# aliftffd/ViT-vs-Raw-IQ

Measured on AMD Instinct MI355X. Metric: IQ frames/sec training (fwd+loss+bwd+clip+AdamW), higher is better.
Workload: dtype bf16; 1 GPU; ViT-Tiny/16 224x224 C=1 19cls (BASELINE configs[1]); config_id=B, per_gpu_batch=256, global_batch=256, parallelism=dp1, hipgraph=True

## Files before the change

vit-vs-raw-iq_amd/csrc/common.h:

```cpp
#pragma once
#include <hip/hip_runtime.h>
#include <stdint.h>

#include "../../include/iqvit.h"

typedef __bf16 bf16;
typedef __attribute__((ext_vector_type(8))) __bf16 bf16x8;
typedef __attribute__((ext_vector_type(4))) __bf16 bf16x4;
typedef __attribute__((ext_vector_type(4))) short s16x4;
typedef __attribute__((ext_vector_type(8))) short s16x8;
typedef __attribute__((ext_vector_type(4))) float f32x4;
typedef __attribute__((ext_vector_type(4))) uint32_t u32x4;
typedef __attribute__((address_space(3))) void lds_void_t;
typedef __attribute__((address_space(1))) const void gbl_cvoid_t;

#define IQ_OK 0
#define IQ_ERR_ARG 1
#define IQ_ERR_UNSUPPORTED 2
#define IQ_ERR_LAUNCH 3

#define IQ_WAVE 64

static inline int iq_launch_status() {
  hipError_t e = hipGetLastError();
  return e == hipSuccess ? IQ_OK : IQ_ERR_LAUNCH;
}

__device__ __forceinline__ float bf2f(bf16 v) { return (float)v; }
__device__ __forceinline__ bf16 f2bf(float v) { return (bf16)v; }

__device__ __forceinline__ void unpack8(const bf16x8& v, float* f) {
#pragma unroll
  for (int i = 0; i < 8; ++i) f[i] = (float)v[i];
}
__device__ __forceinline__ bf16x8 pack8(const float* f) {
  bf16x8 v;
#pragma unroll
  for (int i = 0; i < 8; ++i) v[i] = (bf16)f[i];
  return v;
}

struct IqRng {
  uint64_t seed;
  uint32_t step;
  uint32_t site;
  const uint32_t* step_dev;
};

__device__ __forceinline__ IqRng rng_resolve(IqRng r) {
  if (r.step_dev) r.step = *r.step_dev;
  return r;
}

#ifndef IQ_PHILOX_ROUNDS
#define IQ_PHILOX_ROUNDS 7
#endif
__device__ __forceinline__ u32x4 philox4x32(uint32_t c0, uint32_t c1, uint32_t c2, uint32_t c3,
                                            uint32_t k0, uint32_t k1) {
  const uint32_t M0 = 0xD2511F53u, M1 = 0xCD9E8D57u, W0 = 0x9E3779B9u, W1 = 0xBB67AE85u;
#pragma unroll
  for (int r = 0; r < IQ_PHILOX_ROUNDS; ++r) {
    const uint64_t p0 = (uint64_t)M0 * (uint64_t)c0;
    const uint64_t p1 = (uint64_t)M1 * (uint64_t)c2;
    const uint32_t n0 = (uint32_t)(p1 >> 32) ^ c1 ^ k0, n1 = (uint32_t)p1;
    const uint32_t n2 = (uint32_t)(p0 >> 32) ^ c3 ^ k1, n3 = (uint32_t)p0;
    c0 = n0; c1 = n1; c2 = n2; c3 = n3;
    k0 += W0; k1 += W1;
  }
  u32x4 o = {c0, c1, c2, c3};
  return o;
}

__device__ __forceinline__ float u24(uint32_t w) { return (float)(w >> 8) * 0x1p-24f; }
__device__ __forceinline__ float u24_open(uint32_t w) { return (float)((w >> 8) + 1u) * 0x1p-24f; }
__device__ __forceinline__ void box_muller(uint32_t a, uint32_t b, float& g0, float& g1) {
  const float r = sqrtf(-2.f * logf(u24_open(a)));
  float sn, cs;
  sincospif(2.f * u24(b), &sn, &cs);
  g0 = r * cs;
  g1 = r * sn;
}

__device__ __forceinline__ uint32_t dropout_keep8(const IqRng& r, uint64_t group, uint32_t thresh) {
  u32x4 b = philox4x32((uint32_t)group, (uint32_t)(group >> 32), r.site, r.step,
                          (uint32_t)r.seed, (uint32_t)(r.seed >> 32));
  uint32_t m = 0;
#pragma unroll
  for (int i = 0; i < 4; ++i) {
    m |= ((b[i] & 0xFFFFu) >= thresh ? 1u : 0u) << (2 * i);
    m |= ((b[i] >> 16) >= thresh ? 1u : 0u) << (2 * i + 1);
  }
  return m;
}

__host__ __device__ inline uint32_t dropout_thresh(float p) {
  float t = p * 65536.0f + 0.5f;
  if (t < 0.f) t = 0.f;
  if (t > 65535.f) t = 65535.f;
  return (uint32_t)t;
}
__host__ __device__ inline float dropout_scale(float p) {
  uint32_t t = dropout_thresh(p);
  return 65536.0f / (65536.0f - (float)t);
}

inline bool dropout_unpack(const iq_dropout_t* d, int* on, IqRng* rng, uint32_t* thresh, float* dscale) {
  *on = 0; *rng = IqRng{0, 0, 0, nullptr}; *thresh = 0; *dscale = 1.f;
  if (!d || !(d->p > 0.f)) return true;
  *on = 1;
  *rng = IqRng{d->seed, d->step, d->site, d->step_dev};
  *thresh = dropout_thresh(d->p);
  *dscale = dropout_scale(d->p);
  return d->p < 1.f;
}

constexpr int vmcnt_imm(int n) { return (n & 15) | ((n >> 4) << 14) | 0x0F70; }

__device__ __forceinline__ int xcd_remap(int bid, int nwg) {
  const int NX = 8;
  int q = nwg / NX, r = nwg % NX;
  int xcd = bid % NX, idx = bid / NX;
  int base = (xcd < r) ? xcd * (q + 1) : r * (q + 1) + (xcd - r) * q;
  return base + idx;
}

// ... 11 lines not shown
```

vit-vs-raw-iq_amd/csrc/ffn_chain.hip:

```cpp
#include <stdlib.h>

#include <type_traits>

#include "common.h"
#include "iqvit.h"
#include "prof.h"

namespace {

constexpr int FC_CHUNK = 64, FC_NS = 3, FC_MAXW = 7;

struct FfnChainParams {
  const bf16* X1; const bf16* W1; const bf16* W2;
  const float* b1; const float* b2; const float* gamma; const float* beta;
  bf16* H; bf16* Z; bf16* X; float* mean; float* rstd;
  uint32_t* gate;
  int M, F;
  float eps;
  int drop1_on, drop2_on; IqRng rng1, rng2; uint32_t thresh1, thresh2; float dscale1, dscale2;
  const bf16* A0; const bf16* W0; const bf16* R0; const float* b0; const float* gamma0; const float* beta0;
  bf16* Z0; bf16* X1out; float* mean0; float* rstd0;
  int drop0_on; IqRng rng0; uint32_t thresh0; float dscale0;
  const bf16* Wq; const float* bq; bf16* Yq;
};

template <int CPR> __device__ __forceinline__ int fc_swz(int row, int ch) {
  return CPR == 16 ? (ch ^ (row & 15)) : CPR == 8 ? (ch ^ ((row >> 1) & 7)) : ((ch & ~7) | ((ch & 7) ^ ((row >> 1) & 7)));
}
template <int OFF>
__device__ __forceinline__ void lds_read128(bf16x8& dst, uint32_t addr) {
  asm volatile("ds_read_b128 %0, %1 offset:%2" : "=v"(dst) : "v"(addr), "n"(OFF));
}
#define FC_LGKM_WAIT(N)                                  \
  do {                                                   \
    asm volatile("s_waitcnt lgkmcnt(%0)" ::"n"(N) : "memory"); \
    __builtin_amdgcn_sched_barrier(0);                   \
  } while (0)

__device__ __forceinline__ int fc_kperm(int g) { return ((g & 1) << 1) | (g >> 1); }

template <int D, int NW, int RG, bool DROP1, int MODE>
__global__ __launch_bounds__(NW * 64, 2) void ffn_chain_fwd_kernel(const FfnChainParams p) {
  constexpr int RW = 16 * RG;
  constexpr bool PRE = MODE >= 1, POST = MODE == 2;
  constexpr int XCPR = D / 8;
  constexpr int KS1 = D / 32;
  constexpr int NT2 = D / 16, NP2 = NT2 / 2;
  constexpr int W1_BYTES = FC_CHUNK * D * 2, W2_BYTES = D * FC_CHUNK * 2, SLOT = W1_BYTES + W2_BYTES;
  constexpr int W1_PIECES = W1_BYTES / 1024, PIECES = SLOT / 1024;
  constexpr int PPW = (PIECES + NW - 1) / NW;
  static_assert(PPW + 8 * RG < 64, "counted vmcnt");
  extern __shared__ __attribute__((aligned(16))) unsigned char smem[];
  const int tid = threadIdx.x, lane = tid & 63;
  const int wave = __builtin_amdgcn_readfirstlane(tid >> 6);
  constexpr int nwave = NW;
  const int g = lane >> 4, c16 = lane & 15;
  const bool odd = (g & 1) != 0;
  const int F = p.F;
  const int nchunk = F / FC_CHUNK;
  const long row0 = ((long)blockIdx.x * nwave + wave) * RW;
  const bool have = row0 < p.M;

  auto issue_chunk = [&](int c) {
    unsigned char* slot = smem + (c % FC_NS) * SLOT;
    const char* base1 = reinterpret_cast<const char*>(p.W1 + (long)c * FC_CHUNK * D);
    const char* base2 = reinterpret_cast<const char*>(p.W2 + (long)c * FC_CHUNK);
    int ln = lane;
    asm volatile("" : "+v"(ln));
#pragma unroll
    for (int i = 0; i < PPW; ++i) {
      const int pc = min(wave + i * NW, PIECES - 1);
      const int lin = pc * 64 + ln;
      unsigned off;
      if (pc < W1_PIECES) {
        const int r = lin / XCPR, sl = lin - r * XCPR;
        const int q = fc_swz<XCPR>(r, sl);
        off = (unsigned)((r * D + ((q & ~3) | fc_kperm(q & 3)) * 8) * 2);
      } else {
        const int l2 = lin - W1_PIECES * 64;
        const int r = l2 >> 3, sl = l2 & 7;
        const int q = fc_swz<8>(r, sl);
        off = (unsigned)((r * F + ((q & ~3) | fc_kperm(q & 3)) * 8) * 2);
      }
      const char* base = pc < W1_PIECES ? base1 : base2;
      __builtin_amdgcn_global_load_lds((gbl_cvoid_t*)(base + off), (lds_void_t*)(slot + pc * 1024), 16, 0, 0);
    }
  };
  constexpr int NBQ = 3 * D / FC_CHUNK, NQ = (NBQ + 1) / 2;
  static_assert(2 * W1_BYTES == SLOT, "two projection blocks fill a ring slot");
  const int ntot = nchunk + (POST ? NQ : 0);
  auto issue_any = [&](int c) {
    if (!POST || c < nchunk) { issue_chunk(c); return; }
    const int q = c - nchunk;
    unsigned char* slot = smem + (c % FC_NS) * SLOT;
    int ln = lane;
    asm volatile("" : "+v"(ln));
#pragma unroll
    for (int i = 0; i < PPW; ++i) {
      const int pc = min(wave + i * NW, PIECES - 1);
      const int lin = pc * 64 + ln;
      const int r = lin / XCPR, sl = lin - r * XCPR;
      const int qq = fc_swz<XCPR>(r & 63, sl);
      const int grow = min(q * 2 * FC_CHUNK + r, 3 * D - 1);
      const unsigned off = (unsigned)((grow * D + ((qq & ~3) | fc_kperm(qq & 3)) * 8) * 2);
      __builtin_amdgcn_global_load_lds((gbl_cvoid_t*)(reinterpret_cast<const char*>(p.Wq) + off), (lds_void_t*)(slot + pc * 1024), 16, 0, 0);
    }
  };
  constexpr int NB0 = D / FC_CHUNK;
  if (PRE) {
    constexpr int PRE_PIECES = NB0 * W1_PIECES, PRE_PPW = (PRE_PIECES + NW - 1) / NW;
    static_assert(NB0 * W1_BYTES <= 2 * SLOT, "projection weight blocks fit ring slots 1 and 2");
#pragma unroll
    for (int i = 0; i < PRE_PPW; ++i) {
      const int pc = min(wave + i * NW, PRE_PIECES - 1);
      const int lin = pc * 64 + lane;
      const int r = lin / XCPR, sl = lin - r * XCPR;
      const int q = fc_swz<XCPR>(r & 63, sl);
      const unsigned off = (unsigned)((r * D + ((q & ~3) | fc_kperm(q & 3)) * 8) * 2);
      __builtin_amdgcn_global_load_lds((gbl_cvoid_t*)(reinterpret_cast<const char*>(p.W0) + off),
                                       (lds_void_t*)(smem + SLOT + pc * 1024), 16, 0, 0);
    }
  }
  issue_chunk(0);
  if (!PRE && ntot > 1) issue_any(1);

  bf16x8 xf[RG][KS1];
  {
    const bf16* src = PRE ? p.A0 : p.X1;
#pragma unroll
    for (int rg = 0; rg < RG; ++rg) {
      const long r = min(row0 + rg * 16 + c16, (long)p.M - 1);
#pragma unroll
      for (int ks = 0; ks < KS1; ++ks)
        xf[rg][ks] = have ? *reinterpret_cast<const bf16x8*>(src + r * D + 32 * ks + 8 * fc_kperm(g)) : bf16x8{};
    }
  }
  bf16x8 res0[PRE ? RG : 1][PRE ? KS1 : 1];
  if (PRE) {
#pragma unroll
    for (int rg = 0; rg < RG; ++rg) {
      const long r = min(row0 + rg * 16 + c16, (long)p.M - 1);
#pragma unroll
      for (int jp = 0; jp < KS1; ++jp)
        res0[rg][jp] = have ? *reinterpret_cast<const bf16x8*>(p.R0 + r * D + 32 * jp + 8 * fc_kperm(g)) : bf16x8{};
    }
  }
  const IqRng rng1 = DROP1 ? rng_resolve(p.rng1) : p.rng1;
  const IqRng rng2 = p.drop2_on ? rng_resolve(p.rng2) : p.rng2;
  float* b1s = reinterpret_cast<float*>(smem + FC_NS * SLOT);
  float* vecs = b1s + F;
  for (int i = tid; i < F / 4; i += NW * 64) reinterpret_cast<f32x4*>(b1s)[i] = reinterpret_cast<const f32x4*>(p.b1)[i];
  for (int i = tid; i < (PRE ? 6 : 3) * (D / 4); i += NW * 64) {
    const int v = i / (D / 4), j = i - v * (D / 4);
    const float* src = v == 0 ? p.b2 : v == 1 ? p.gamma : v == 2 ? p.beta : v == 3 ? p.b0 : v == 4 ? p.gamma0 : p.beta0;
    reinterpret_cast<f32x4*>(vecs)[i] = reinterpret_cast<const f32x4*>(src)[j];
  }
  if (POST)
    for (int i = tid; i < 3 * D / 4; i += NW * 64) reinterpret_cast<f32x4*>(vecs + 6 * D)[i] = reinterpret_cast<const f32x4*>(p.bq)[i];
  asm volatile("s_waitcnt vmcnt(0)" ::: "memory");
#pragma unroll
  for (int rg = 0; rg < RG; ++rg)
#pragma unroll
    for (int ks = 0; ks < KS1; ++ks) asm volatile("" : "+v"(xf[rg][ks]));
  if (PRE) {
#pragma unroll
    for (int rg = 0; rg < RG; ++rg)
#pragma unroll
      for (int jp = 0; jp < KS1; ++jp) asm volatile("" : "+v"(res0[rg][jp]));
  }

  const uint32_t lds0 = (uint32_t)(uintptr_t)(lds_void_t*)smem;
  constexpr int W1_KMASK = XCPR == 24 ? 1 : KS1 - 1;
  uint32_t w1off[KS1], w2off[2];
  auto w1at = [&](int ks) -> uint32_t { return w1off[ks & W1_KMASK] + (XCPR == 24 ? 128u * (uint32_t)(ks >> 1) : 0u); };
#pragma unroll
  for (int ks = 0; ks < KS1; ++ks) w1off[ks] = (uint32_t)(c16 * (D * 2) + fc_swz<XCPR>(c16, 4 * (ks & W1_KMASK) + g) * 16);
#pragma unroll
  for (int jp = 0; jp < 2; ++jp) w2off[jp] = (uint32_t)(W1_BYTES + c16 * 128 + fc_swz<8>(c16, 4 * jp + g) * 16);

  if (PRE) {
    __syncthreads();
    if (have) {
      const IqRng rng0 = p.drop0_on ? rng_resolve(p.rng0) : p.rng0;
      bf16x8 zb[RG][KS1];
#pragma unroll
      for (int b = 0; b < NB0; ++b) {
#pragma unroll
        for (int jp = 0; jp < 2; ++jp) {
          const int col = 32 * (2 * b + jp) + (odd ? 16 + 4 * (g - 1) : 4 * g);
          f32x4 acc1[RG][2];
#pragma unroll
          for (int rg = 0; rg < RG; ++rg) { acc1[rg][0] = f32x4{0.f, 0.f, 0.f, 0.f}; acc1[rg][1] = f32x4{0.f, 0.f, 0.f, 0.f}; }
          bf16x8 wp[2][2];
          const uint32_t blk = lds0 + SLOT + b * W1_BYTES;
          auto read_w0 = [&](int ks, bf16x8 (&dst)[2]) {
            const uint32_t a0 = blk + w1at(ks);
            if (jp == 0) { lds_read128<0 * 16 * D * 2>(dst[0], a0); lds_read128<1 * 16 * D * 2>(dst[1], a0); }
            else { lds_read128<2 * 16 * D * 2>(dst[0], a0); lds_read128<3 * 16 * D * 2>(dst[1], a0); }
          };
          read_w0(0, wp[0]);
#pragma unroll
          for (int ks = 0; ks < KS1; ++ks) {
            if (ks + 1 < KS1) { read_w0(ks + 1, wp[(ks + 1) & 1]); FC_LGKM_WAIT(2); }
            else FC_LGKM_WAIT(0);
#pragma unroll
            for (int t = 0; t < 2; ++t) {
#pragma unroll
              for (int rg = 0; rg < RG; ++rg)
                acc1[rg][t] = __builtin_amdgcn_mfma_f32_16x16x32_bf16(wp[ks & 1][t], xf[rg][ks], acc1[rg][t], 0, 0, 0);
            }
            __builtin_amdgcn_sched_barrier(0);
          }
          const f32x4 b_lo = *reinterpret_cast<const f32x4*>(vecs + 3 * D + col), b_hi = *reinterpret_cast<const f32x4*>(vecs + 3 * D + col + 4);
#pragma unroll
          for (int rg = 0; rg < RG; ++rg) {
            float w[8];
#pragma unroll
            for (int r = 0; r < 4; ++r) {
              const float va = acc1[rg][0][r], vb = acc1[rg][1][r];
              const auto sw = __builtin_amdgcn_permlane16_swap(__float_as_uint(va), __float_as_uint(vb), false, false);
              w[r] = __uint_as_float(sw[0]) + b_lo[r];
              w[4 + r] = __uint_as_float(sw[1]) + b_hi[r];
            }
            const long grow = row0 + rg * 16 + c16;
            if (p.drop0_on) {
              const uint32_t keep = dropout_keep8(rng0, (uint64_t)(grow * D + col) >> 3, p.thresh0);
#pragma unroll
              for (int e = 0; e < 8; ++e) w[e] = ((keep >> e) & 1u) ? w[e] * p.dscale0 : 0.f;
            }
#pragma unroll
            for (int e = 0; e < 8; ++e) w[e] += (float)res0[rg][2 * b + jp][e];
            zb[rg][2 * b + jp] = pack8(w);
            if (grow < p.M) *reinterpret_cast<bf16x8*>(p.Z0 + grow * D + col) = zb[rg][2 * b + jp];
          }
        }
      }
      const float invD0 = 1.0f / (float)D;
#pragma unroll
      for (int rg = 0; rg < RG; ++rg) {
        const long grow = row0 + rg * 16 + c16;
        float s1 = 0.f;
#pragma unroll
        for (int jp = 0; jp < KS1; ++jp)
#pragma unroll
          for (int e = 0; e < 8; ++e) s1 += (float)zb[rg][jp][e];
        s1 += __shfl_xor(s1, 16, 64);
        s1 += __shfl_xor(s1, 32, 64);
        const float mean = s1 * invD0;
        float s2 = 0.f;
#pragma unroll
        for (int jp = 0; jp < KS1; ++jp)
#pragma unroll
          for (int e = 0; e < 8; ++e) { const float d = (float)zb[rg][jp][e] - mean; s2 += d * d; }
        s2 += __shfl_xor(s2, 16, 64);
        s2 += __shfl_xor(s2, 32, 64);
        const float rstd = 1.0f / sqrtf(s2 * invD0 + p.eps);
        if (g == 0 && grow < p.M) { p.mean0[grow] = mean; p.rstd0[grow] = rstd; }
#pragma unroll
        for (int jp = 0; jp < KS1; ++jp) {
// ... 59 lines not shown
        else { lds_read128<2 * 16 * D * 2>(dst[0], a0); lds_read128<3 * 16 * D * 2>(dst[1], a0); }
      };
      read_w1(0, wp[0]);
#pragma unroll
      for (int ks = 0; ks < KS1; ++ks) {
        if (ks + 1 < KS1) { read_w1(ks + 1, wp[(ks + 1) & 1]); FC_LGKM_WAIT(2); }
        else FC_LGKM_WAIT(0);
#pragma unroll
        for (int t = 0; t < 2; ++t) {
#ifdef FC_NO_MFMA
          asm volatile("" :: "v"(wp[ks & 1][t]));
#else
#pragma unroll
          for (int rg = 0; rg < RG; ++rg)
            acc1[rg][t] = __builtin_amdgcn_mfma_f32_16x16x32_bf16(wp[ks & 1][t], xf[rg][ks], acc1[rg][t], 0, 0, 0);
#endif
        }
        __builtin_amdgcn_sched_barrier(0);
      }
      const int col = f0 + 32 * jp + (odd ? 16 + 4 * (g - 1) : 4 * g);
      const f32x4 b_lo = *reinterpret_cast<const f32x4*>(b1s + col), b_hi = *reinterpret_cast<const f32x4*>(b1s + col + 4);
#pragma unroll
      for (int rg = 0; rg < RG; ++rg) {
        float w[8];
#pragma unroll
        for (int r = 0; r < 4; ++r) {
          const float va = acc1[rg][0][r], vb = acc1[rg][1][r];
          const auto sw = __builtin_amdgcn_permlane16_swap(__float_as_uint(va), __float_as_uint(vb), false, false);
          w[r] = fmaxf(__uint_as_float(sw[0]) + b_lo[r], 0.f);
          w[4 + r] = fmaxf(__uint_as_float(sw[1]) + b_hi[r], 0.f);
        }
        const long grow = row0 + rg * 16 + c16;
        if (DROP1) {
          const uint32_t keep = dropout_keep8(rng1, (uint64_t)(grow * F + col) >> 3, p.thresh1);
#pragma unroll
          for (int e = 0; e < 8; ++e) w[e] = ((keep >> e) & 1u) ? w[e] * p.dscale1 : 0.f;
        }
        hf[rg][jp] = pack8(w);
#pragma unroll
        for (int e = 0; e < 8; ++e) gbits |= (w[e] > 0.f ? 1u : 0u) << (8 * (2 * jp + rg) + e);
#ifndef FC_NO_HSTORE
        if (grow < p.M) *reinterpret_cast<bf16x8*>(p.H + grow * F + col) = hf[rg][jp];
#endif
      }
    }
    {
      if (gated) p.gate[((row0 / RW) * nchunk + c) * 64 + lane] = gbits;
    }
    constexpr int NG4 = NT2 / 4, NGRP = 2 * NG4;
    bf16x8 wq[2][4];
    auto read_w2 = [&](auto qc, bf16x8 (&dst)[4]) {
      constexpr int q = decltype(qc)::value;
      constexpr int jp = q / NG4, j0 = 4 * (q % NG4);
      const uint32_t a0 = slot_addr + w2off[jp];
      lds_read128<(j0 + 0) * 16 * 128>(dst[0], a0);
      lds_read128<(j0 + 1) * 16 * 128>(dst[1], a0);
      lds_read128<(j0 + 2) * 16 * 128>(dst[2], a0);
      lds_read128<(j0 + 3) * 16 * 128>(dst[3], a0);
    };
    auto p2 = [&](auto self, auto qc) -> void {
      constexpr int q = decltype(qc)::value;
      if constexpr (q < NGRP) {
        if constexpr (q + 1 < NGRP) { read_w2(std::integral_constant<int, q + 1>{}, wq[(q + 1) & 1]); FC_LGKM_WAIT(4); }
        else FC_LGKM_WAIT(0);
        constexpr int jp = q / NG4, j0 = 4 * (q % NG4);
#pragma unroll
        for (int t = 0; t < 4; ++t) {
#ifdef FC_NO_MFMA
          asm volatile("" :: "v"(wq[q & 1][t]), "v"(hf[0][jp]), "v"(hf[RG - 1][jp]));
#else
#pragma unroll
          for (int rg = 0; rg < RG; ++rg)
            acc2[rg][j0 + t] = __builtin_amdgcn_mfma_f32_16x16x32_bf16(wq[q & 1][t], hf[rg][jp], acc2[rg][j0 + t], 0, 0, 0);
#endif
        }
        __builtin_amdgcn_sched_barrier(0);
        self(self, std::integral_constant<int, q + 1>{});
      }
    };
    read_w2(std::integral_constant<int, 0>{}, wq[0]);
    p2(p2, std::integral_constant<int, 0>{});
  }
  if (!POST && !have) return;

  const float invD = 1.0f / (float)D;
  if (have) {
#pragma unroll
  for (int rg = 0; rg < RG; ++rg) {
    const long grow = row0 + rg * 16 + c16;
    float z[NP2][8];
    float s1 = 0.f;
#pragma unroll
    for (int jp = 0; jp < NP2; ++jp) {
      const int col = 32 * jp + (odd ? 16 + 4 * (g - 1) : 4 * g);
      const f32x4 b_lo = *reinterpret_cast<const f32x4*>(vecs + col), b_hi = *reinterpret_cast<const f32x4*>(vecs + col + 4);
      float w[8];
#pragma unroll
      for (int r = 0; r < 4; ++r) {
        const float va = acc2[rg][2 * jp][r], vb = acc2[rg][2 * jp + 1][r];
        const auto sw = __builtin_amdgcn_permlane16_swap(__float_as_uint(va), __float_as_uint(vb), false, false);
        w[r] = __uint_as_float(sw[0]) + b_lo[r];
        w[4 + r] = __uint_as_float(sw[1]) + b_hi[r];
      }
      if (p.drop2_on) {
        const uint32_t keep = dropout_keep8(rng2, (uint64_t)(grow * D + col) >> 3, p.thresh2);
#pragma unroll
        for (int e = 0; e < 8; ++e) w[e] = ((keep >> e) & 1u) ? w[e] * p.dscale2 : 0.f;
      }
#pragma unroll
      for (int e = 0; e < 8; ++e) w[e] += (float)xf[rg][jp][e];
      const bf16x8 zb = pack8(w);
      if (grow < p.M) *reinterpret_cast<bf16x8*>(p.Z + grow * D + col) = zb;
      unpack8(zb, z[jp]);
#pragma unroll
      for (int e = 0; e < 8; ++e) s1 += z[jp][e];
    }
    s1 += __shfl_xor(s1, 16, 64);
    s1 += __shfl_xor(s1, 32, 64);
    const float mean = s1 * invD;
    float s2 = 0.f;
#pragma unroll
    for (int jp = 0; jp < NP2; ++jp)
#pragma unroll
      for (int e = 0; e < 8; ++e) { const float d = z[jp][e] - mean; s2 += d * d; }
    s2 += __shfl_xor(s2, 16, 64);
    s2 += __shfl_xor(s2, 32, 64);
    const float rstd = 1.0f / sqrtf(s2 * invD + p.eps);
    if (grow < p.M) {
      if (g == 0) { p.mean[grow] = mean; p.rstd[grow] = rstd; }
#pragma unroll
      for (int jp = 0; jp < NP2; ++jp) {
        const int col = 32 * jp + (odd ? 16 + 4 * (g - 1) : 4 * g);
        const f32x4 g_lo = *reinterpret_cast<const f32x4*>(vecs + D + col), g_hi = *reinterpret_cast<const f32x4*>(vecs + D + col + 4);
        const f32x4 e_lo = *reinterpret_cast<const f32x4*>(vecs + 2 * D + col), e_hi = *reinterpret_cast<const f32x4*>(vecs + 2 * D + col + 4);
        float y[8];
#pragma unroll
        for (int e = 0; e < 4; ++e) {
          y[e] = g_lo[e] * ((z[jp][e] - mean) * rstd) + e_lo[e];
          y[4 + e] = g_hi[e] * ((z[jp][4 + e] - mean) * rstd) + e_hi[e];
        }
        const bf16x8 yb = pack8(y);
        *reinterpret_cast<bf16x8*>(p.X + grow * D + col) = yb;
        if (POST) xf[rg][jp] = yb;
      }
    }
  }
  }
  if (!POST) return;

  for (int q = 0; q < NQ; ++q) {
    const int c = nchunk + q;
    if (q == 0 || !full) asm volatile("s_waitcnt vmcnt(0)" ::: "memory");
    else if (c + 1 < ntot) asm volatile("s_waitcnt vmcnt(%0)" :: "n"(PPW + 8 * RG) : "memory");
    else asm volatile("s_waitcnt vmcnt(%0)" :: "n"(8 * RG) : "memory");
    __builtin_amdgcn_s_barrier();
    asm volatile("" ::: "memory");
    if (c + 2 < ntot) issue_any(c + 2);
    if (!have) continue;
    const uint32_t slot_addr = lds0 + (c % FC_NS) * SLOT;
#pragma unroll
    for (int bl = 0; bl < 2; ++bl) {
      if (2 * q + bl >= NBQ) break;
#pragma unroll
      for (int jp = 0; jp < 2; ++jp) {
        f32x4 acc1[RG][2];
#pragma unroll
        for (int rg = 0; rg < RG; ++rg) { acc1[rg][0] = f32x4{0.f, 0.f, 0.f, 0.f}; acc1[rg][1] = f32x4{0.f, 0.f, 0.f, 0.f}; }
        bf16x8 wp[2][2];
        const uint32_t blk = slot_addr + bl * W1_BYTES;
        auto read_wq = [&](int ks, bf16x8 (&dst)[2]) {
          const uint32_t a0 = blk + w1at(ks);
          if (jp == 0) { lds_read128<0 * 16 * D * 2>(dst[0], a0); lds_read128<1 * 16 * D * 2>(dst[1], a0); }
          else { lds_read128<2 * 16 * D * 2>(dst[0], a0); lds_read128<3 * 16 * D * 2>(dst[1], a0); }
        };
        read_wq(0, wp[0]);
#pragma unroll
        for (int ks = 0; ks < KS1; ++ks) {
          if (ks + 1 < KS1) { read_wq(ks + 1, wp[(ks + 1) & 1]); FC_LGKM_WAIT(2); }
          else FC_LGKM_WAIT(0);
#pragma unroll
          for (int t = 0; t < 2; ++t) {
#pragma unroll
            for (int rg = 0; rg < RG; ++rg)
              acc1[rg][t] = __builtin_amdgcn_mfma_f32_16x16x32_bf16(wp[ks & 1][t], xf[rg][ks], acc1[rg][t], 0, 0, 0);
          }
          __builtin_amdgcn_sched_barrier(0);
        }
        const int col = FC_CHUNK * (2 * q + bl) + 32 * jp + (odd ? 16 + 4 * (g - 1) : 4 * g);
        const f32x4 b_lo = *reinterpret_cast<const f32x4*>(vecs + 6 * D + col), b_hi = *reinterpret_cast<const f32x4*>(vecs + 6 * D + col + 4);
#pragma unroll
        for (int rg = 0; rg < RG; ++rg) {
          float w[8];
#pragma unroll
          for (int r = 0; r < 4; ++r) {
            const float va = acc1[rg][0][r], vb = acc1[rg][1][r];
            const auto sw = __builtin_amdgcn_permlane16_swap(__float_as_uint(va), __float_as_uint(vb), false, false);
            w[r] = __uint_as_float(sw[0]) + b_lo[r];
            w[4 + r] = __uint_as_float(sw[1]) + b_hi[r];
          }
          const long grow = row0 + rg * 16 + c16;
          if (grow < p.M) *reinterpret_cast<bf16x8*>(p.Yq + grow * (3 * D) + col) = pack8(w);
        }
      }
    }
  }
}

struct FfnChainBwdParams {
  const bf16* dO; const bf16* W2t; const bf16* W1t;
  const uint32_t* gate; const bf16* R; const bf16* Z1;
  const float* mean; const float* rstd; const float* gamma;
  bf16* gH; bf16* dZ; bf16* dY; float* partial;
  int M, F;
  float gate_scale;
  int drop_on; IqRng rng; uint32_t thresh; float dscale;
  const bf16* Wot; bf16* dA;
  const bf16* A0; const bf16* W0t; const bf16* R0; const bf16* Z0; const float* mean0; const float* rstd0; const float* gamma0;
  IqRng rng0; bf16* dZ0; bf16* dY0; float* partial0;
};

template <int D, int NW, int RG, bool DROP, int MODE>
__global__ __launch_bounds__(NW * 64, 2) void ffn_chain_bwd_kernel(const FfnChainBwdParams p) {
  constexpr int RW = 16 * RG;
  constexpr bool POSTB = MODE >= 1, PREB = MODE == 2;
  constexpr int XCPR = D / 8;
  constexpr int KS1 = D / 32;
  constexpr int NT2 = D / 16, NP2 = NT2 / 2;
  constexpr int W1_BYTES = FC_CHUNK * D * 2, W2_BYTES = D * FC_CHUNK * 2, SLOT = W1_BYTES + W2_BYTES;
  constexpr int W1_PIECES = W1_BYTES / 1024, PIECES = SLOT / 1024;
  constexpr int PPW = (PIECES + NW - 1) / NW;
  extern __shared__ __attribute__((aligned(16))) unsigned char smem[];
  const int tid = threadIdx.x, lane = tid & 63;
  const int wave = __builtin_amdgcn_readfirstlane(tid >> 6);
// ... 412 lines not shown
        else { lds_read128<2 * 16 * D * 2>(dst[0], a0); lds_read128<3 * 16 * D * 2>(dst[1], a0); }
      };
      read_w(0, wp[0]);
#pragma unroll
      for (int ks = 0; ks < KS1; ++ks) {
        if (ks + 1 < KS1) { read_w(ks + 1, wp[(ks + 1) & 1]); FC_LGKM_WAIT(2); }
        else FC_LGKM_WAIT(0);
#pragma unroll
        for (int t = 0; t < 2; ++t) {
#pragma unroll
          for (int rg = 0; rg < RG; ++rg)
            acc1[rg][t] = __builtin_amdgcn_mfma_f32_16x16x32_bf16(wp[ks & 1][t], xf[rg][ks], acc1[rg][t], 0, 0, 0);
        }
        __builtin_amdgcn_sched_barrier(0);
      }
      const int col = FC_CHUNK * b + 32 * jp + (odd ? 16 + 4 * (g - 1) : 4 * g);
#pragma unroll
      for (int rg = 0; rg < RG; ++rg) {
        float w[8];
#pragma unroll
        for (int r = 0; r < 4; ++r) {
          const float va = acc1[rg][0][r], vb = acc1[rg][1][r];
          const auto sw = __builtin_amdgcn_permlane16_swap(__float_as_uint(va), __float_as_uint(vb), false, false);
          w[r] = __uint_as_float(sw[0]);
          w[4 + r] = __uint_as_float(sw[1]);
        }
        const long grow = row0 + rg * 16 + c16;
        if (grow < p.M) *reinterpret_cast<bf16x8*>(p.dA + grow * D + col) = pack8(w);
      }
    }
  }
}

struct ChainShape { int rg, nw; };
inline ChainShape chain_shape(int M) {
  if (M <= 20480) return ChainShape{1, 5};
  if (M <= 32768) return ChainShape{1, 8};
  return ChainShape{2, FC_MAXW};
}
inline int chain_waves(int M) { return chain_shape(M).nw; }
inline long chain_units(int M) { const int rw = 16 * chain_shape(M).rg; return ((long)M + rw - 1) / rw; }

template <int D, int NW, int RG>
int launch_chain(const FfnChainParams& p, hipStream_t st) {
  constexpr int SLOT = 2 * FC_CHUNK * D * 2;
  const size_t lds = (size_t)FC_NS * SLOT + ((size_t)p.F + 9 * D) * sizeof(float);
  const long units = ((long)p.M + 16 * RG - 1) / (16 * RG);
  const int grid = (int)((units + NW - 1) / NW);
#define FC_LAUNCH(DROP_, MODE_)                                                                                               \
  do {                                                                                                                        \
    auto k = ffn_chain_fwd_kernel<D, NW, RG, DROP_, MODE_>;                                                                   \
    static const hipError_t attr = hipFuncSetAttribute((const void*)k, hipFuncAttributeMaxDynamicSharedMemorySize, 160 * 1024); \
    (void)attr;                                                                                                               \
    k<<<grid, NW * 64, lds, st>>>(p);                                                                                         \
  } while (0)
  if (p.A0 && p.Wq) { if (p.drop1_on) FC_LAUNCH(true, 2); else FC_LAUNCH(false, 2); }
  else if (p.A0) { if (p.drop1_on) FC_LAUNCH(true, 1); else FC_LAUNCH(false, 1); }
  else { if (p.drop1_on) FC_LAUNCH(true, 0); else FC_LAUNCH(false, 0); }
#undef FC_LAUNCH
  return iq_launch_status();
}
template <int D>
int launch_chain_d(const FfnChainParams& p, hipStream_t st) {
  const ChainShape sh = chain_shape(p.M);
  if (sh.rg == 2) return launch_chain<D, FC_MAXW, 2>(p, st);
  return sh.nw == 5 ? launch_chain<D, 5, 1>(p, st) : launch_chain<D, 8, 1>(p, st);
}

template <int D, int NW, int RG>
int launch_chain_bwd(const FfnChainBwdParams& p, hipStream_t st) {
  constexpr int SLOT = 2 * FC_CHUNK * D * 2;
  const size_t lds = (size_t)FC_NS * SLOT + (size_t)NW * 2 * D * sizeof(float);
  const long units = ((long)p.M + 16 * RG - 1) / (16 * RG);
  const int grid = (int)((units + NW - 1) / NW);
#define FC_LAUNCHB(DROP_, MODE_)                                                                                              \
  do {                                                                                                                        \
    auto k = ffn_chain_bwd_kernel<D, NW, RG, DROP_, MODE_>;                                                                   \
    static const hipError_t attr = hipFuncSetAttribute((const void*)k, hipFuncAttributeMaxDynamicSharedMemorySize, 160 * 1024); \
    (void)attr;                                                                                                               \
    k<<<grid, NW * 64, lds, st>>>(p);                                                                                         \
  } while (0)
  if (p.A0) { if (p.drop_on) FC_LAUNCHB(true, 2); else FC_LAUNCHB(false, 2); }
  else if (p.Wot) { if (p.drop_on) FC_LAUNCHB(true, 1); else FC_LAUNCHB(false, 1); }
  else { if (p.drop_on) FC_LAUNCHB(true, 0); else FC_LAUNCHB(false, 0); }
#undef FC_LAUNCHB
  return iq_launch_status();
}
template <int D>
int launch_chain_bwd_d(const FfnChainBwdParams& p, hipStream_t st) {
  const ChainShape sh = chain_shape(p.M);
  if (sh.rg == 2) return launch_chain_bwd<D, FC_MAXW, 2>(p, st);
  return sh.nw == 5 ? launch_chain_bwd<D, 5, 1>(p, st) : launch_chain_bwd<D, 8, 1>(p, st);
}

}

extern "C" int iq_ffn_chain_supported(int S, int D, int F) {
  if (!(D == 128 || D == 192) || F < FC_CHUNK || (F % FC_CHUNK) || S <= 0) return 0;
  return (size_t)FC_NS * 2 * FC_CHUNK * D * 2 + ((size_t)F + 9 * D) * sizeof(float) <= (size_t)160 * 1024 ? 1 : 0;
}

namespace {
struct ChainPre {
  const void* A0; const void* W0; const float* b0; const iq_dropout_t* drop0; const void* R0;
  const float* gamma0; const float* beta0; void* Z0; float* mean0; float* rstd0;
  const void* Wq; const float* bq; void* Yq;
};

int chain_fwd(const ChainPre* pre, const void* X1, const void* W1, const float* b1, const iq_dropout_t* drop1, void* H, const void* W2,
              const float* b2, const iq_dropout_t* drop2, const float* gamma, const float* beta, float eps, void* Z, void* X,
              float* mean, float* rstd, void* gate_bits, int frames, int S, int D, int F, iq_stream_t stream) {
  if (frames <= 0) return IQ_OK;
  if (!X1 || !W1 || !b1 || !H || !W2 || !b2 || !gamma || !beta || !Z || !X || !mean || !rstd) return IQ_ERR_ARG;
  if (!iq_ffn_chain_supported(S, D, F)) return IQ_ERR_UNSUPPORTED;
  if (((uintptr_t)X1 | (uintptr_t)W1 | (uintptr_t)W2 | (uintptr_t)H | (uintptr_t)Z | (uintptr_t)X | (uintptr_t)b1 | (uintptr_t)b2 |
       (uintptr_t)gamma | (uintptr_t)beta) % 16) return IQ_ERR_ARG;
  if ((long)frames * S > 0x7FFFFFFFL) return IQ_ERR_UNSUPPORTED;
  FfnChainParams p = {};
  p.X1 = (const bf16*)X1; p.W1 = (const bf16*)W1; p.W2 = (const bf16*)W2;
  p.b1 = b1; p.b2 = b2; p.gamma = gamma; p.beta = beta;
  p.H = (bf16*)H; p.Z = (bf16*)Z; p.X = (bf16*)X; p.mean = mean; p.rstd = rstd;
  p.gate = (uint32_t*)gate_bits;
  if ((uintptr_t)gate_bits % 16) return IQ_ERR_ARG;
  p.M = frames * S; p.F = F; p.eps = eps;
  if (!dropout_unpack(drop1, &p.drop1_on, &p.rng1, &p.thresh1, &p.dscale1) ||
      !dropout_unpack(drop2, &p.drop2_on, &p.rng2, &p.thresh2, &p.dscale2)) return IQ_ERR_ARG;
  if (pre) {
    if (!pre->A0 || !pre->W0 || !pre->b0 || !pre->R0 || !pre->gamma0 || !pre->beta0 || !pre->Z0 || !pre->mean0 || !pre->rstd0)
      return IQ_ERR_ARG;
    if (((uintptr_t)pre->A0 | (uintptr_t)pre->W0 | (uintptr_t)pre->b0 | (uintptr_t)pre->R0 | (uintptr_t)pre->gamma0 |
         (uintptr_t)pre->beta0 | (uintptr_t)pre->Z0) % 16) return IQ_ERR_ARG;
    p.A0 = (const bf16*)pre->A0; p.W0 = (const bf16*)pre->W0; p.R0 = (const bf16*)pre->R0; p.b0 = pre->b0;
    p.gamma0 = pre->gamma0; p.beta0 = pre->beta0; p.Z0 = (bf16*)pre->Z0; p.X1out = (bf16*)X1; p.mean0 = pre->mean0; p.rstd0 = pre->rstd0;
    if (!dropout_unpack(pre->drop0, &p.drop0_on, &p.rng0, &p.thresh0, &p.dscale0)) return IQ_ERR_ARG;
    if (pre->Wq || pre->bq || pre->Yq) {
      if (!pre->Wq || !pre->bq || !pre->Yq || ((uintptr_t)pre->Wq | (uintptr_t)pre->bq | (uintptr_t)pre->Yq) % 16) return IQ_ERR_ARG;
      p.Wq = (const bf16*)pre->Wq; p.bq = pre->bq; p.Yq = (bf16*)pre->Yq;
    }
  }
  hipStream_t st = (hipStream_t)stream;
  IQ_PROF(IQ_FAM_GEMM_NT, st);
  const double M = (double)p.M;
  double more_bytes = 0.0, more_flops = 0.0;
  if (pre) { more_bytes += 2.0 * (M * D * 3 + (double)D * D) + 8.0 * M; more_flops += 2.0 * M * D * D; }
  if (p.Wq) { more_bytes += 2.0 * (M * 3 * D + 3.0 * D * D); more_flops += 6.0 * M * D * D; }
  IQ_PROF_K(2.0 * (M * D * 3 + M * F + 2.0 * D * F) + 8.0 * M + more_bytes, 4.0 * M * D * F + more_flops,
            "ffn_chain_fwd_kernel<%d, %d, %d, %s, %d>", D, chain_waves(p.M), chain_shape(p.M).rg, p.drop1_on ? "true" : "false", p.Wq ? 2 : pre ? 1 : 0);
  return D == 192 ? launch_chain_d<192>(p, st) : launch_chain_d<128>(p, st);
}
}

extern "C" int iq_ffn_chain_fwd(const void* X1, const void* W1, const float* b1, const iq_dropout_t* drop1, void* H,
                                const void* W2, const float* b2, const iq_dropout_t* drop2, const float* gamma,
                                const float* beta, float eps, void* Z, void* X, float* mean, float* rstd, void* gate_bits,
                                int frames, int S, int D, int F, iq_stream_t stream) {
  return chain_fwd(nullptr, X1, W1, b1, drop1, H, W2, b2, drop2, gamma, beta, eps, Z, X, mean, rstd, gate_bits, frames, S, D, F, stream);
}
// ... 93 lines not shown
```

Baseline: 52740 frames/s.

## Precompute ring-load offsets in LDS and hoist uniform Philox rounds for dropout

Per-lane swizzled global offsets for the W1/W2/Wq/W0 weight-ring loads are now computed once into a small LDS class table and reused as a base plus a per-piece step, so the repeated index arithmetic in each chunk issue goes away. The dropout Philox generator also gets a 'head' form: when row*cols fits in 32 bits, the parts of the first two rounds that depend only on seed, site and step are computed once per kernel, leaving fewer multiplies per 8-element mask. The cost is extra LDS for the table, a tighter LDS-capacity check, and more register and scheduling pressure from the hand-unrolled rounds.

After: 52830 frames/s, median of 6. No clear change (+0.2%).

```diff
diff --git a/vit-vs-raw-iq_amd/csrc/chain_ring.h b/vit-vs-raw-iq_amd/csrc/chain_ring.h
--- /dev/null
+++ b/vit-vs-raw-iq_amd/csrc/chain_ring.h
@@ -0,0 +1,39 @@
+#pragma once
+
+#if defined(__HIPCC__)
+#define FC_HD __host__ __device__ inline __attribute__((always_inline))
+#else
+#define FC_HD inline
+#endif
+
+template <int CPR> FC_HD int fc_swz(int row, int ch) {
+  return CPR == 16 ? (ch ^ (row & 15)) : CPR == 8 ? (ch ^ ((row >> 1) & 7)) : ((ch & ~7) | ((ch & 7) ^ ((row >> 1) & 7)));
+}
+FC_HD int fc_kperm(int g) { return ((g & 1) << 1) | (g >> 1); }
+
+template <int D> FC_HD unsigned fc_w1_off(int lin) {
+  constexpr int XCPR = D / 8;
+  const int r = lin / XCPR, sl = lin - r * XCPR;
+  const int q = fc_swz<XCPR>(r, sl);
+  return (unsigned)((r * D + ((q & ~3) | fc_kperm(q & 3)) * 8) * 2);
+}
+FC_HD unsigned fc_w2_off(int lin, int F) {
+  const int r = lin >> 3, sl = lin & 7;
+  const int q = fc_swz<8>(r, sl);
+  return (unsigned)((r * F + ((q & ~3) | fc_kperm(q & 3)) * 8) * 2);
+}
+
+template <int D> FC_HD int fc_w1_class(int pc) { return (int)((unsigned)pc % (D / 32u)); }
+template <int D> FC_HD unsigned fc_w1_step(int pc) { return (unsigned)pc / (D / 32u) * (16u * D * 2u); }
+template <int D> FC_HD int fc_w2_class(int pc) { return D / 32 + (pc & 1); }
+FC_HD unsigned fc_w2_step(int pc, int F) { return ((unsigned)pc >> 1) * (32u * (unsigned)F); }
+template <int D> constexpr int fc_classes() { return D / 32 + 2; }
+
+FC_HD int fc_piece(int wave, int i, int nw, int pieces) {
+  const int pc = wave + i * nw;
+  return (nw - 1 + i * nw < pieces || pc < pieces) ? pc : pieces - 1;
+}
+FC_HD bool fc_piece_in_w1(int pc, int i, int nw, int w1_pieces) {
+  return nw - 1 + i * nw < w1_pieces || (i * nw < w1_pieces && pc < w1_pieces);
+}
+FC_HD int fc_post_src_piece(int pc, int w1_pieces, bool half) { return half && pc >= w1_pieces ? pc - w1_pieces : pc; }
diff --git a/vit-vs-raw-iq_amd/csrc/common.h b/vit-vs-raw-iq_amd/csrc/common.h
--- a/vit-vs-raw-iq_amd/csrc/common.h
+++ b/vit-vs-raw-iq_amd/csrc/common.h
@@ -55,8 +55,8 @@
 #ifndef IQ_PHILOX_ROUNDS
 #define IQ_PHILOX_ROUNDS 7
 #endif
-__device__ __forceinline__ u32x4 philox4x32(uint32_t c0, uint32_t c1, uint32_t c2, uint32_t c3,
-                                            uint32_t k0, uint32_t k1) {
+__host__ __device__ __forceinline__ u32x4 philox4x32(uint32_t c0, uint32_t c1, uint32_t c2, uint32_t c3,
+                                                     uint32_t k0, uint32_t k1) {
   const uint32_t M0 = 0xD2511F53u, M1 = 0xCD9E8D57u, W0 = 0x9E3779B9u, W1 = 0xBB67AE85u;
 #pragma unroll
   for (int r = 0; r < IQ_PHILOX_ROUNDS; ++r) {
@@ -81,9 +81,7 @@
   g1 = r * sn;
 }
 
-__device__ __forceinline__ uint32_t dropout_keep8(const IqRng& r, uint64_t group, uint32_t thresh) {
-  u32x4 b = philox4x32((uint32_t)group, (uint32_t)(group >> 32), r.site, r.step,
-                          (uint32_t)r.seed, (uint32_t)(r.seed >> 32));
+__host__ __device__ __forceinline__ uint32_t keep8_bits(const u32x4& b, uint32_t thresh) {
   uint32_t m = 0;
 #pragma unroll
   for (int i = 0; i < 4; ++i) {
@@ -91,6 +89,49 @@
     m |= ((b[i] >> 16) >= thresh ? 1u : 0u) << (2 * i + 1);
   }
   return m;
+}
+__host__ __device__ __forceinline__ uint32_t dropout_keep8(const IqRng& r, uint64_t group, uint32_t thresh) {
+  u32x4 b = philox4x32((uint32_t)group, (uint32_t)(group >> 32), r.site, r.step,
+                          (uint32_t)r.seed, (uint32_t)(r.seed >> 32));
+  return keep8_bits(b, thresh);
+}
+
+struct IqRngHead {
+  uint32_t r1_lo, r1_hi;
+  uint32_t r2_lo, r2_hi;
+};
+__host__ __device__ __forceinline__ IqRngHead rng_head(const IqRng& r) {
+  const uint64_t p1 = (uint64_t)0xCD9E8D57u * (uint64_t)r.site;
+  const uint32_t c0 = (uint32_t)(p1 >> 32) ^ (uint32_t)r.seed;
+  const uint64_t p0 = (uint64_t)0xD2511F53u * (uint64_t)c0;
+  return IqRngHead{(uint32_t)p1, (uint32_t)(p1 >> 32), (uint32_t)p0, (uint32_t)(p0 >> 32)};
+}
+__host__ __device__ __forceinline__ u32x4 philox4x32_head(uint32_t group_lo, const IqRng& r, const IqRngHead& h) {
+  static_assert(IQ_PHILOX_ROUNDS >= 2, "two rounds are unrolled by hand");
+  const uint32_t M0 = 0xD2511F53u, M1 = 0xCD9E8D57u, W0 = 0x9E3779B9u, W1 = 0xBB67AE85u;
+  uint32_t k0 = (uint32_t)r.seed, k1 = (uint32_t)(r.seed >> 32);
+  const uint64_t a0 = (uint64_t)M0 * (uint64_t)group_lo;
+  const uint32_t a_n1 = h.r1_lo, a_n2 = (uint32_t)(a0 >> 32) ^ r.step ^ k1, a_n3 = (uint32_t)a0;
+  k0 += W0; k1 += W1;
+  const uint64_t b1 = (uint64_t)M1 * (uint64_t)a_n2;
+  uint32_t c0 = (uint32_t)(b1 >> 32) ^ a_n1 ^ k0, c1 = (uint32_t)b1, c2 = h.r2_hi ^ a_n3 ^ k1, c3 = h.r2_lo;
+  k0 += W0; k1 += W1;
+#pragma unroll
+  for (int rd = 2; rd < IQ_PHILOX_ROUNDS; ++rd) {
+    const uint64_t p0 = (uint64_t)M0 * (uint64_t)c0;
+    const uint64_t p1 = (uint64_t)M1 * (uint64_t)c2;
+    const uint32_t n0 = (uint32_t)(p1 >> 32) ^ c1 ^ k0, n1 = (uint32_t)p1;
+    const uint32_t n2 = (uint32_t)(p0 >> 32) ^ c3 ^ k1, n3 = (uint32_t)p0;
+    c0 = n0; c1 = n1; c2 = n2; c3 = n3;
+    k0 += W0; k1 += W1;
+  }
+  u32x4 o = {c0, c1, c2, c3};
+  return o;
+}
+__host__ __device__ __forceinline__ uint32_t dropout_keep8_head(const IqRng& r, const IqRngHead& h, bool lo32, uint64_t group,
+                                                                uint32_t thresh) {
+  if (!lo32) return dropout_keep8(r, group, thresh);
+  return keep8_bits(philox4x32_head((uint32_t)group, r, h), thresh);
 }
 
 __host__ __device__ inline uint32_t dropout_thresh(float p) {
diff --git a/vit-vs-raw-iq_amd/csrc/ffn_chain.hip b/vit-vs-raw-iq_amd/csrc/ffn_chain.hip
--- a/vit-vs-raw-iq_amd/csrc/ffn_chain.hip
+++ b/vit-vs-raw-iq_amd/csrc/ffn_chain.hip
@@ -2,6 +2,7 @@
 
 #include <type_traits>
 
+#include "chain_ring.h"
 #include "common.h"
 #include "iqvit.h"
 #include "prof.h"
@@ -9,6 +10,10 @@
 namespace {
 
 constexpr int FC_CHUNK = 64, FC_NS = 3, FC_MAXW = 7;
+
+#ifndef FC_PHILOX_HEAD
+#define FC_PHILOX_HEAD 1
+#endif
 
 struct FfnChainParams {
   const bf16* X1; const bf16* W1; const bf16* W2;
@@ -18,15 +23,13 @@
   int M, F;
   float eps;
   int drop1_on, drop2_on; IqRng rng1, rng2; uint32_t thresh1, thresh2; float dscale1, dscale2;
+  int drop_lo32;
   const bf16* A0; const bf16* W0; const bf16* R0; const float* b0; const float* gamma0; const float* beta0;
   bf16* Z0; bf16* X1out; float* mean0; float* rstd0;
   int drop0_on; IqRng rng0; uint32_t thresh0; float dscale0;
   const bf16* Wq; const float* bq; bf16* Yq;
 };
 
-template <int CPR> __device__ __forceinline__ int fc_swz(int row, int ch) {
-  return CPR == 16 ? (ch ^ (row & 15)) : CPR == 8 ? (ch ^ ((row >> 1) & 7)) : ((ch & ~7) | ((ch & 7) ^ ((row >> 1) & 7)));
-}
 template <int OFF>
 __device__ __forceinline__ void lds_read128(bf16x8& dst, uint32_t addr) {
   asm volatile("ds_read_b128 %0, %1 offset:%2" : "=v"(dst) : "v"(addr), "n"(OFF));
@@ -37,7 +40,12 @@
     __builtin_amdgcn_sched_barrier(0);                   \
   } while (0)
 
-__device__ __forceinline__ int fc_kperm(int g) { return ((g & 1) << 1) | (g >> 1); }
+
+__device__ __forceinline__ IqRng fc_rng_resolve(IqRng r) {
+  r = rng_resolve(r);
+  r.step = __builtin_amdgcn_readfirstlane(r.step);
+  return r;
+}
 
 template <int D, int NW, int RG, bool DROP1, int MODE>
 __global__ __launch_bounds__(NW * 64, 2) void ffn_chain_fwd_kernel(const FfnChainParams p) {
@@ -61,29 +69,38 @@
   const long row0 = ((long)blockIdx.x * nwave + wave) * RW;
   const bool have = row0 < p.M;
 
+  constexpr int NC1 = D / 32;
+  uint32_t* ctab = reinterpret_cast<uint32_t*>(smem + FC_NS * SLOT) + F + 9 * D;
+#pragma unroll
+  for (int k = 0; k < NC1; ++k) ctab[k * 64 + lane] = fc_w1_off<D>(k * 64 + lane);
+#pragma unroll
+  for (int k = 0; k < 2; ++k) ctab[(NC1 + k) * 64 + lane] = fc_w2_off(k * 64 + lane, F);
+  static_assert(W1_PIECES % NC1 == 0, "an image starts a class period");
+  typedef __attribute__((address_space(3))) const uint32_t lds_cu32_t;
+  auto ring_wave = [&]() { int w = wave; asm volatile("" : "+s"(w)); return w; };
+  auto ring_offsets = [&](auto cls_of, uint32_t (&voff)[PPW]) {
+    int ln = lane;
+    asm volatile("" : "+v"(ln));
+#pragma unroll
+    for (int i = 0; i < PPW; ++i) voff[i] = ((lds_cu32_t*)(lds_void_t*)ctab)[cls_of(i) * 64 + ln];
+#pragma unroll
+    for (int i = 0; i < PPW; ++i) asm volatile("" : "+v"(voff[i]));
+  };
   auto issue_chunk = [&](int c) {
     unsigned char* slot = smem + (c % FC_NS) * SLOT;
     const char* base1 = reinterpret_cast<const char*>(p.W1 + (long)c * FC_CHUNK * D);
     const char* base2 = reinterpret_cast<const char*>(p.W2 + (long)c * FC_CHUNK);
-    int ln = lane;
-    asm volatile("" : "+v"(ln));
+    const int wv = ring_wave();
+    uint32_t voff[PPW];
+    ring_offsets([&](int i) {
+      const int pc = fc_piece(wv, i, NW, PIECES);
+      return fc_piece_in_w1(pc, i, NW, W1_PIECES) ? fc_w1_class<D>(pc) : fc_w2_class<D>(pc - W1_PIECES);
+    }, voff);
 #pragma unroll
     for (int i = 0; i < PPW; ++i) {
-      const int pc = min(wave + i * NW, PIECES - 1);
-      const int lin = pc * 64 + ln;
-      unsigned off;
-      if (pc < W1_PIECES) {
-        const int r = lin / XCPR, sl = lin - r * XCPR;
-        const int q = fc_swz<XCPR>(r, sl);
-        off = (unsigned)((r * D + ((q & ~3) | fc_kperm(q & 3)) * 8) * 2);
-      } else {
-        const int l2 = lin - W1_PIECES * 64;
-        const int r = l2 >> 3, sl = l2 & 7;
-        const int q = fc_swz<8>(r, sl);
-        off = (unsigned)((r * F + ((q & ~3) | fc_kperm(q & 3)) * 8) * 2);
-      }
-      const char* base = pc < W1_PIECES ? base1 : base2;
-      __builtin_amdgcn_global_load_lds((gbl_cvoid_t*)(base + off), (lds_void_t*)(slot + pc * 1024), 16, 0, 0);
+      const int pc = fc_piece(wv, i, NW, PIECES);
+      const char* src = fc_piece_in_w1(pc, i, NW, W1_PIECES) ? base1 + fc_w1_step<D>(pc) : base2 + fc_w2_step(pc - W1_PIECES, F);
+      __builtin_amdgcn_global_load_lds((gbl_cvoid_t*)(src + voff[i]), (lds_void_t*)(slot + pc * 1024), 16, 0, 0);
     }
   };
   constexpr int NBQ = 3 * D / FC_CHUNK, NQ = (NBQ + 1) / 2;
@@ -93,17 +110,16 @@
     if (!POST || c < nchunk) { issue_chunk(c); return; }
     const int q = c - nchunk;
     unsigned char* slot = smem + (c % FC_NS) * SLOT;
-    int ln = lane;
-    asm volatile("" : "+v"(ln));
+    const char* base = reinterpret_cast<const char*>(p.Wq + (long)q * 2 * FC_CHUNK * D);
+    const bool half = 2 * q + 1 >= NBQ;
+    const int wv = ring_wave();
+    uint32_t voff[PPW];
+    ring_offsets([&](int i) { return fc_w1_class<D>(fc_piece(wv, i, NW, PIECES)); }, voff);
 #pragma unroll
     for (int i = 0; i < PPW; ++i) {
-      const int pc = min(wave + i * NW, PIECES - 1);
-      const int lin = pc * 64 + ln;
-      const int r = lin / XCPR, sl = lin - r * XCPR;
-      const int qq = fc_swz<XCPR>(r & 63, sl);
-      const int grow = min(q * 2 * FC_CHUNK + r, 3 * D - 1);
-      const unsigned off = (unsigned)((grow * D + ((qq & ~3) | fc_kperm(qq & 3)) * 8) * 2);
-      __builtin_amdgcn_global_load_lds((gbl_cvoid_t*)(reinterpret_cast<const char*>(p.Wq) + off), (lds_void_t*)(slot + pc * 1024), 16, 0, 0);
+      const int pc = fc_piece(wv, i, NW, PIECES);
+      const int ps = fc_post_src_piece(pc, W1_PIECES, half);
+      __builtin_amdgcn_global_load_lds((gbl_cvoid_t*)(base + fc_w1_step<D>(ps) + voff[i]), (lds_void_t*)(slot + pc * 1024), 16, 0, 0);
     }
   };
   constexpr int NB0 = D / FC_CHUNK;
@@ -112,12 +128,10 @@
     static_assert(NB0 * W1_BYTES <= 2 * SLOT, "projection weight blocks fit ring slots 1 and 2");
 #pragma unroll
     for (int i = 0; i < PRE_PPW; ++i) {
-      const int pc = min(wave + i * NW, PRE_PIECES - 1);
-      const int lin = pc * 64 + lane;
-      const int r = lin / XCPR, sl = lin - r * XCPR;
-      const int q = fc_swz<XCPR>(r & 63, sl);
-      const unsigned off = (unsigned)((r * D + ((q & ~3) | fc_kperm(q & 3)) * 8) * 2);
-      __builtin_amdgcn_global_load_lds((gbl_cvoid_t*)(reinterpret_cast<const char*>(p.W0) + off),
+      const int pc = fc_piece(wave, i, NW, PRE_PIECES);
+      uint32_t voff = ctab[fc_w1_class<D>(pc) * 64 + lane];
+      asm volatile("" : "+v"(voff));
+      __builtin_amdgcn_global_load_lds((gbl_cvoid_t*)(reinterpret_cast<const char*>(p.W0) + fc_w1_step<D>(pc) + voff),
                                        (lds_void_t*)(smem + SLOT + pc * 1024), 16, 0, 0);
     }
   }
@@ -145,8 +159,10 @@
         res0[rg][jp] = have ? *reinterpret_cast<const bf16x8*>(p.R0 + r * D + 32 * jp + 8 * fc_kperm(g)) : bf16x8{};
     }
   }
-  const IqRng rng1 = DROP1 ? rng_resolve(p.rng1) : p.rng1;
-  const IqRng rng2 = p.drop2_on ? rng_resolve(p.rng2) : p.rng2;
+  const IqRng rng1 = DROP1 ? fc_rng_resolve(p.rng1) : p.rng1;
+  const IqRng rng2 = p.drop2_on ? fc_rng_resolve(p.rng2) : p.rng2;
+  const IqRngHead head1 = rng_head(rng1), head2 = rng_head(rng2);
+  const bool lo32 = FC_PHILOX_HEAD && p.drop_lo32 != 0;
   float* b1s = reinterpret_cast<float*>(smem + FC_NS * SLOT);
   float* vecs = b1s + F;
   for (int i = tid; i < F / 4; i += NW * 64) reinterpret_cast<f32x4*>(b1s)[i] = reinterpret_cast<const f32x4*>(p.b1)[i];
@@ -181,7 +197,8 @@
   if (PRE) {
     __syncthreads();
     if (have) {
-      const IqRng rng0 = p.drop0_on ? rng_resolve(p.rng0) : p.rng0;
+      const IqRng rng0 = p.drop0_on ? fc_rng_resolve(p.rng0) : p.rng0;
+      const IqRngHead head0 = rng_head(rng0);
       bf16x8 zb[RG][KS1];
 #pragma unroll
       for (int b = 0; b < NB0; ++b) {
@@ -224,7 +241,7 @@
             }
             const long grow = row0 + rg * 16 + c16;
             if (p.drop0_on) {
-              const uint32_t keep = dropout_keep8(rng0, (uint64_t)(grow * D + col) >> 3, p.thresh0);
+              const uint32_t keep = dropout_keep8_head(rng0, head0, lo32, (uint64_t)(grow * D + col) >> 3, p.thresh0);
 #pragma unroll
               for (int e = 0; e < 8; ++e) w[e] = ((keep >> e) & 1u) ? w[e] * p.dscale0 : 0.f;
             }
@@ -350,7 +367,7 @@
         }
         const long grow = row0 + rg * 16 + c16;
         if (DROP1) {
-          const uint32_t keep = dropout_keep8(rng1, (uint64_t)(grow * F + col) >> 3, p.thresh1);
+          const uint32_t keep = dropout_keep8_head(rng1, head1, lo32, (uint64_t)(grow * F + col) >> 3, p.thresh1);
 #pragma unroll
           for (int e = 0; e < 8; ++e) w[e] = ((keep >> e) & 1u) ? w[e] * p.dscale1 : 0.f;
         }
@@ -403,6 +420,10 @@
 
   const float invD = 1.0f / (float)D;
   if (have) {
+  int lane_t = lane;
+  asm volatile("" : "+v"(lane_t));
+  const int g = lane_t >> 4, c16 = lane_t & 15;
+  const bool odd = (g & 1) != 0;
 #pragma unroll
   for (int rg = 0; rg < RG; ++rg) {
     const long grow = row0 + rg * 16 + c16;
@@ -421,7 +442,7 @@
         w[4 + r] = __uint_as_float(sw[1]) + b_hi[r];
       }
       if (p.drop2_on) {
-        const uint32_t keep = dropout_keep8(rng2, (uint64_t)(grow * D + col) >> 3, p.thresh2);
+        const uint32_t keep = dropout_keep8_head(rng2, head2, lo32, (uint64_t)(grow * D + col) >> 3, p.thresh2);
 #pragma unroll
         for (int e = 0; e < 8; ++e) w[e] = ((keep >> e) & 1u) ? w[e] * p.dscale2 : 0.f;
       }
@@ -466,6 +487,9 @@
   }
   if (!POST) return;
 
+  int lane_q = lane;
+  asm volatile("" : "+v"(lane_q));
+  const int gq = lane_q >> 4, c16q = lane_q & 15;
   for (int q = 0; q < NQ; ++q) {
     const int c = nchunk + q;
     if (q == 0 || !full) asm volatile("s_waitcnt vmcnt(0)" ::: "memory");
@@ -504,7 +528,7 @@
           }
           __builtin_amdgcn_sched_barrier(0);
         }
-        const int col = FC_CHUNK * (2 * q + bl) + 32 * jp + (odd ? 16 + 4 * (g - 1) : 4 * g);
+        const int col = FC_CHUNK * (2 * q + bl) + 32 * jp + ((gq & 1) ? 16 + 4 * (gq - 1) : 4 * gq);
         const f32x4 b_lo = *reinterpret_cast<const f32x4*>(vecs + 6 * D + col), b_hi = *reinterpret_cast<const f32x4*>(vecs + 6 * D + col + 4);
 #pragma unroll
         for (int rg = 0; rg < RG; ++rg) {
@@ -516,7 +540,7 @@
             w[r] = __uint_as_float(sw[0]) + b_lo[r];
             w[4 + r] = __uint_as_float(sw[1]) + b_hi[r];
           }
-          const long grow = row0 + rg * 16 + c16;
+          const long grow = row0 + rg * 16 + c16q;
           if (grow < p.M) *reinterpret_cast<bf16x8*>(p.Yq + grow * (3 * D) + col) = pack8(w);
         }
       }
@@ -995,19 +1019,21 @@
   }
 }
 
+inline size_t chain_class_bytes(int D) { return (size_t)(D / 32 + 2) * 64 * sizeof(uint32_t); }
 struct ChainShape { int rg, nw; };
 inline ChainShape chain_shape(int M) {
   if (M <= 20480) return ChainShape{1, 5};
   if (M <= 32768) return ChainShape{1, 8};
   return ChainShape{2, FC_MAXW};
 }
+inline int chain_drop_lo32(int M, int D, int F) { return ((long)M + 32) * (long)(F > D ? F : D) <= (1L << 35) ? 1 : 0; }
 inline int chain_waves(int M) { return chain_shape(M).nw; }
 inline long chain_units(int M) { const int rw = 16 * chain_shape(M).rg; return ((long)M + rw - 1) / rw; }
 
 template <int D, int NW, int RG>
 int launch_chain(const FfnChainParams& p, hipStream_t st) {
   constexpr int SLOT = 2 * FC_CHUNK * D * 2;
-  const size_t lds = (size_t)FC_NS * SLOT + ((size_t)p.F + 9 * D) * sizeof(float);
+  const size_t lds = (size_t)FC_NS * SLOT + ((size_t)p.F + 9 * D) * sizeof(float) + chain_class_bytes(D);
   const long units = ((long)p.M + 16 * RG - 1) / (16 * RG);
   const int grid = (int)((units + NW - 1) / NW);
 #define FC_LAUNCH(DROP_, MODE_)                                                                                               \
@@ -1060,7 +1086,7 @@
 
 extern "C" int iq_ffn_chain_supported(int S, int D, int F) {
   if (!(D == 128 || D == 192) || F < FC_CHUNK || (F % FC_CHUNK) || S <= 0) return 0;
-  return (size_t)FC_NS * 2 * FC_CHUNK * D * 2 + ((size_t)F + 9 * D) * sizeof(float) <= (size_t)160 * 1024 ? 1 : 0;
+  return (size_t)FC_NS * 2 * FC_CHUNK * D * 2 + ((size_t)F + 9 * D) * sizeof(float) + chain_class_bytes(D) <= (size_t)160 * 1024 ? 1 : 0;
 }
 
 namespace {
@@ -1086,6 +1112,7 @@
   p.gate = (uint32_t*)gate_bits;
   if ((uintptr_t)gate_bits % 16) return IQ_ERR_ARG;
   p.M = frames * S; p.F = F; p.eps = eps;
+  p.drop_lo32 = chain_drop_lo32(p.M, D, F);
   if (!dropout_unpack(drop1, &p.drop1_on, &p.rng1, &p.thresh1, &p.dscale1) ||
       !dropout_unpack(drop2, &p.drop2_on, &p.rng2, &p.thresh2, &p.dscale2)) return IQ_ERR_ARG;
   if (pre) {
```
